# ctu-mrs/space_filling_forest_star

Measured on AMD Instinct MI355X. Metric: accepted node expansions/sec + collision checks/sec, dense_3D 6-DoF, higher is better.
Workload: dtype f64

## Files before the change

### space_filling_forest_star_amd/csrc/engine.cpp

```cpp
#include "engine.h"
#include <dlfcn.h>

#include <algorithm>
#include <chrono>
#include <cmath>
#include <cstdlib>
#include <cstring>
#include <limits>

#include "sff_geom.h"

namespace sff {

void hip_check(hipError_t e, const char* what) {
  if (e != hipSuccess) throw HipError{std::string(what) + ": " + hipGetErrorString(e)};
}
#define HIPCHK(x) hip_check((x), #x)

void DevBuf::ensure(size_t bytes) {
  if (bytes <= cap) return;
  size_t want = std::max(bytes, cap * 2);
  want = (want + 255) & ~(size_t)255;
  void* np = nullptr;
  HIPCHK(hipMalloc(&np, want));
// ... 142 lines not shown
  HIPCHK(hipEventCreateWithFlags(&ev_mid, hipEventDisableTiming));
  HIPCHK(hipEventCreateWithFlags(&ev_early, hipEventDisableTiming));
}

namespace {
struct RcclApi {
  struct Id128 { char b[128]; };
  int (*GetUniqueId)(void*) = nullptr;
  int (*CommInitRank)(void**, int, Id128, int) = nullptr;
  int (*AllGather)(const void*, void*, size_t, int, void*, hipStream_t) = nullptr;
  int (*CommDestroy)(void*) = nullptr;
  const char* (*GetErrorString)(int) = nullptr;
  bool ok = false;
};
RcclApi& rccl() {
  static RcclApi api;
  static bool tried = false;
  if (tried) return api;
  tried = true;
  void* h = nullptr;
  for (const char* name : {"librccl.so.1", "librccl.so"}) {
    h = dlopen(name, RTLD_NOW | RTLD_NOLOAD);
    if (h) break;
  }
  for (const char* name : {"librccl.so.1", "librccl.so", "/opt/rocm/lib/librccl.so.1"}) {
    if (h) break;
    h = dlopen(name, RTLD_NOW | RTLD_GLOBAL);
  }
  if (!h) return api;
  api.GetUniqueId = reinterpret_cast<decltype(api.GetUniqueId)>(dlsym(h, "ncclGetUniqueId"));
  api.CommInitRank = reinterpret_cast<decltype(api.CommInitRank)>(dlsym(h, "ncclCommInitRank"));
  api.AllGather = reinterpret_cast<decltype(api.AllGather)>(dlsym(h, "ncclAllGather"));
  api.CommDestroy = reinterpret_cast<decltype(api.CommDestroy)>(dlsym(h, "ncclCommDestroy"));
  api.GetErrorString = reinterpret_cast<decltype(api.GetErrorString)>(dlsym(h, "ncclGetErrorString"));
  api.ok = api.GetUniqueId && api.CommInitRank && api.AllGather && api.CommDestroy;
  return api;
}
void rccl_check(int rc, const char* what) {
  if (rc == 0) return;
  const char* msg = rccl().GetErrorString ? rccl().GetErrorString(rc) : "?";
  throw HipError{std::string("rccl: ") + what + " failed: " + msg};
}
}

void Ctx::rccl_unique_id(uint8_t* id128) {
  if (!rccl().ok) throw HipError{"rccl: librccl could not be bound"};
  rccl_check(rccl().GetUniqueId(id128), "ncclGetUniqueId");
}
void Ctx::rccl_init(const uint8_t* id128, int rank, int world) {
  if (!rccl().ok) throw HipError{"rccl: librccl could not be bound"};
  if (world < 1 || rank < 0 || rank >= world) throw HipError{"rccl: bad rank / world"};
  HIPCHK(hipSetDevice(device));
  if (rccl_comm) { (void)rccl().CommDestroy(rccl_comm); rccl_comm = nullptr; }
  RcclApi::Id128 id;
  memcpy(id.b, id128, 128);
  rccl_check(rccl().CommInitRank(&rccl_comm, world, id, rank), "ncclCommInitRank");
  rccl_rank = rank;
  rccl_world = world;
}
void Ctx::rccl_all_gather_i32(const void* send, void* recv, size_t words) {
  if (xchg_fn) {
    if (xchg_fn(xchg_user, send, recv, words, stream) != 0) throw HipError{"exchange: the caller's all-gather failed"};
    return;
  }
  rccl_check(rccl().AllGather(send, recv, words,  2, rccl_comm, stream), "ncclAllGather");
}

Ctx::~Ctx() {
  (void)hipSetDevice(device);
  if (stream) (void)hipStreamSynchronize(stream);
  if (own_stream && own_stream != stream) (void)hipStreamSynchronize(own_stream);
  if (copy_stream) (void)hipStreamSynchronize(copy_stream);
  if (rccl_comm && rccl().CommDestroy) { (void)rccl().CommDestroy(rccl_comm); rccl_comm = nullptr; }
  for (hipEvent_t e : rr_ev) if (e) (void)hipEventDestroy(e);
  for (SegJob& J : seg_job) if (J.ev) (void)hipEventDestroy(J.ev);
  if (ev_mid) (void)hipEventDestroy(ev_mid);
  if (ev_early) (void)hipEventDestroy(ev_early);
  for (auto& t : pending) { (void)hipEventDestroy(t.a); (void)hipEventDestroy(t.b); }
  for (auto e : pool) (void)hipEventDestroy(e);
  DevBuf* bufs[] = {&env_tri, &env_box, &env_plane, &rob_tri, &sx, &sy, &sz, &syaw, &spitch, &sroll, &stree, &spos,
                    &d_a, &d_b, &d_c, &d_d, &d_e, &d_f, &d_g, &d_h, &r_in, &r_out, &r_out2, &r_q, &r_cnt, &r_hidx,
                    &r_hdist, &r_sega, &r_segb, &r_items, &r_items2, &r_center, &r_qrec, &env_clear, &env_clear_edge, &env_cand, &g_cnt, &g_items, &g_ovfcnt, &g_ovf, &t_cnt, &t_items, &t_ovfcnt, &t_ovf, &t_occ, &g_lite, &g_ovf_lite, &t_lite, &t_ovf_lite, &env_tg_start, &env_tg_list, &r_sub, &env_ext, &rr_q1, &rr_q2, &rr_a, &rr_out, &rr_sq, &rr_np, &rr_alt, &rr_q2b, &rr_sqb, &seg_job[0].ids, &seg_job[0].a, &seg_job[0].b, &seg_job[0].c, &seg_job[1].ids, &seg_job[1].a,
                    &seg_job[1].b, &seg_job[1].c, &seg_job[2].ids, &seg_job[2].a, &seg_job[2].b, &seg_job[2].c, &seg_job[3].ids, &seg_job[3].a,
                    &seg_job[3].b, &seg_job[3].c};
  for (DevBuf* b : bufs) b->release();
  for (auto& b : level_box) b.release();
  PinBuf* pins[] = {&h_a, &h_b, &h_c, &h_d, &h_e, &h_f, &h_g, &h_h, &p_in, &p_out, &rr_hq, &rr_hout, &seg_job[0].hids, &seg_job[0].hc, &seg_job[1].hids, &seg_job[1].hc, &seg_job[2].hids, &seg_job[2].hc,
                    &seg_job[3].hids, &seg_job[3].hc};
  for (PinBuf* b : pins) b->release();
  if (copy_stream) (void)hipStreamDestroy(copy_stream);
  if (own_stream) (void)hipStreamDestroy(own_stream);
}

void Ctx::set_stream(hipStream_t s) {
  HIPCHK(hipSetDevice(device));
  sync();
  stream = s ? s : own_stream;
}

hipEvent_t Ctx::get_event() {
  if (!pool.empty()) {
    hipEvent_t e = pool.back();
    pool.pop_back();
    return e;
  }
  hipEvent_t e;
  HIPCHK(hipEventCreate(&e));
  return e;
}
void Ctx::time_begin(int kind) {
  kernel_calls[kind] += 1;
  if (round_scope) round_calls[kind] += 1;
  timed_now = timing_on;
  if (!timed_now) return;
  Timed t{get_event(), get_event(), kind, round_scope};
  HIPCHK(hipEventRecord(t.a, stream));
  pending.push_back(t);
}
void Ctx::time_end() { if (timed_now) HIPCHK(hipEventRecord(pending.back().b, stream)); }
double Ctx::kernel_ms_total(int kind) const {
  double ms = kernel_ms[kind];
  if (round_timed[kind]) ms += round_ms[kind] * ((double)round_calls[kind] / (double)round_timed[kind]);
  return ms;
}
void Ctx::sync() {
  HIPCHK(hipStreamSynchronize(stream));
  for (auto& t : pending) {
    float ms = 0;
    HIPCHK(hipEventElapsedTime(&ms, t.a, t.b));
    if (t.round) { round_ms[t.kind] += ms; round_timed[t.kind] += 1; }
    else kernel_ms[t.kind] += ms;
    kernel_launches[t.kind] += 1;
    pool.push_back(t.a);
    pool.push_back(t.b);
  }
  pending.clear();
}

static inline uint64_t spread21(uint64_t v) {
  v &= 0x1FFFFF;
  v = (v | v << 32) & 0x1F00000000FFFFULL;
  v = (v | v << 16) & 0x1F0000FF0000FFULL;
  v = (v | v << 8) & 0x100F00F00F00F00FULL;
  v = (v | v << 4) & 0x10C30C30C30C30C3ULL;
  v = (v | v << 2) & 0x1249249249249249ULL;
  return v;
}

void Ctx::upload_mesh(int role, const double* tri9, int n) {
  kn = Knobs::from_env();
  HIPCHK(hipSetDevice(device));
  if (role == SFFGPU_MESH_ROBOT) {
    if (n <= 0) throw HipError{"robot mesh must have at least one triangle"};
    rob_tri.ensure((size_t)n * 9 * sizeof(double));
    HIPCHK(hipMemcpy(rob_tri.p, tri9, (size_t)n * 9 * sizeof(double), hipMemcpyHostToDevice));
    robv.tri = rob_tri.as<double>();
    robv.n_tri = n;
    double lo[3] = {1e300, 1e300, 1e300}, hi[3] = {-1e300, -1e300, -1e300};
    for (int v = 0; v < n * 3; ++v)
      for (int i = 0; i < 3; ++i) {
        lo[i] = std::min(lo[i], tri9[3 * v + i]);
        hi[i] = std::max(hi[i], tri9[3 * v + i]);
      }
    double rad = 0;
    for (int i = 0; i < 3; ++i) { robv.lo[i] = lo[i]; robv.hi[i] = hi[i]; robv.center[i] = 0.5 * (lo[i] + hi[i]); }
    for (int v = 0; v < n * 3; ++v) {
      double d2 = 0;
      for (int i = 0; i < 3; ++i) d2 += (tri9[3 * v + i] - robv.center[i]) * (tri9[3 * v + i] - robv.center[i]);
      rad = std::max(rad, std::sqrt(d2));
    }
    robv.radius = rad;
    have_robot = true;
    h_rob.assign(tri9, tri9 + (size_t)n * 9);
    build_robot_extents();
    build_clearance();
    build_tri_grid();
    return;
  }
  if (role != SFFGPU_MESH_ENV) throw HipError{"unknown mesh role"};
  envv = sffk::EnvView{};
  have_env = true;
  clear_cells = 0;
  if (n <= 0) return;
  std::vector<double> box((size_t)n * 6);
  double glo[3] = {1e300, 1e300, 1e300}, ghi[3] = {-1e300, -1e300, -1e300};
  for (int t = 0; t < n; ++t)
    for (int a = 0; a < 3; ++a) {
      const double* P = tri9 + 9 * (size_t)t;
      double lo = std::min(P[a], std::min(P[3 + a], P[6 + a])), hi = std::max(P[a], std::max(P[3 + a], P[6 + a]));
      box[6 * (size_t)t + a] = lo;
      box[6 * (size_t)t + 3 + a] = hi;
      glo[a] = std::min(glo[a], lo);
      ghi[a] = std::max(ghi[a], hi);
    }
  for (int a = 0; a < 3; ++a) { env_lo[a] = glo[a]; env_hi[a] = ghi[a]; }
  env_maxabs = 1.0;
  for (int a = 0; a < 3; ++a) env_maxabs = std::max(env_maxabs, std::max(std::fabs(glo[a]), std::fabs(ghi[a])));
  std::vector<std::pair<uint64_t, int>> order(n);
  for (int t = 0; t < n; ++t) {
    uint64_t code = 0;
    for (int a = 0; a < 3; ++a) {
      double ext = ghi[a] - glo[a];
      double c = 0.5 * (box[6 * (size_t)t + a] + box[6 * (size_t)t + 3 + a]);
      double u = ext > 0 ? (c - glo[a]) / ext : 0.0;
      uint64_t q = (uint64_t)std::min(2097151.0, std::max(0.0, u * 2097151.0));
      code |= spread21(q) << a;
    }
    order[t] = {code, t};
  }
  std::sort(order.begin(), order.end());
  std::vector<double> tri_s((size_t)n * 9), box_s((size_t)n * 6);
  for (int k = 0; k < n; ++k) {
    memcpy(&tri_s[9 * (size_t)k], tri9 + 9 * (size_t)order[k].second, 9 * sizeof(double));
    memcpy(&box_s[6 * (size_t)k], &box[6 * (size_t)order[k].second], 6 * sizeof(double));
  }
  env_tri.ensure(tri_s.size() * sizeof(double));
  env_box.ensure(box_s.size() * sizeof(double));
  HIPCHK(hipMemcpy(env_tri.p, tri_s.data(), tri_s.size() * sizeof(double), hipMemcpyHostToDevice));
  HIPCHK(hipMemcpy(env_box.p, box_s.data(), box_s.size() * sizeof(double), hipMemcpyHostToDevice));
  std::vector<double> plane((size_t)n * 5);
  for (int k = 0; k < n; ++k) {
    const double* P = &tri_s[9 * (size_t)k];
    double e1[3] = {P[3] - P[0], P[4] - P[1], P[5] - P[2]}, e2[3] = {P[6] - P[0], P[7] - P[1], P[8] - P[2]}, nn[3];
    sffg::cross(e1, e2, nn);
    plane[5 * (size_t)k + 0] = nn[0];
    plane[5 * (size_t)k + 1] = nn[1];
    plane[5 * (size_t)k + 2] = nn[2];
    plane[5 * (size_t)k + 3] = (nn[0] * P[0] + nn[1] * P[1]) + nn[2] * P[2];
    plane[5 * (size_t)k + 4] = std::sqrt(nn[0] * nn[0] + nn[1] * nn[1] + nn[2] * nn[2]);
  }
  env_plane.ensure(plane.size() * sizeof(double));
  HIPCHK(hipMemcpy(env_plane.p, plane.data(), plane.size() * sizeof(double), hipMemcpyHostToDevice));
  envv.tri = env_tri.as<double>();
  envv.tri_box = env_box.as<double>();
  envv.tri_plane = env_plane.as<double>();
  envv.n_tri = n;
  h_plane = plane;
  std::vector<double> cur = box_s;
  int count = n, L = 0;
  while (true) {
    int groups = (count + 63) / 64;
    std::vector<double> nxt((size_t)groups * 6);
    for (int g = 0; g < groups; ++g) {
      double lo[3] = {1e300, 1e300, 1e300}, hi[3] = {-1e300, -1e300, -1e300};
      for (int k = g * 64; k < std::min(count, g * 64 + 64); ++k)
        for (int a = 0; a < 3; ++a) {
          lo[a] = std::min(lo[a], cur[6 * (size_t)k + a]);
          hi[a] = std::max(hi[a], cur[6 * (size_t)k + 3 + a]);
        }
      for (int a = 0; a < 3; ++a) { nxt[6 * (size_t)g + a] = lo[a]; nxt[6 * (size_t)g + 3 + a] = hi[a]; }
    }
    if (L >= SFFK_MAX_LEVELS) throw HipError{"environment mesh too large for the box hierarchy"};
    level_box[L].ensure(nxt.size() * sizeof(double));
    HIPCHK(hipMemcpy(level_box[L].p, nxt.data(), nxt.size() * sizeof(double), hipMemcpyHostToDevice));
    envv.level_box[L] = level_box[L].as<double>();
    envv.level_count[L] = groups;
    ++L;
    cur.swap(nxt);
    count = groups;
    if (groups <= 64) break;
  }
  envv.n_levels = L;
  build_robot_extents();
  build_clearance();
  build_tri_grid();
}

void Ctx::build_robot_extents() {
  envv.tri_ext = nullptr;
  envv.cand = nullptr;
  if (!have_env || !have_robot || envv.n_tri <= 0 || h_rob.empty() || h_plane.size() != (size_t)envv.n_tri * 5) return;
  std::vector<double> ext((size_t)envv.n_tri * 2);
  const size_t nv = h_rob.size() / 3;
  for (int k = 0; k < envv.n_tri; ++k) {
    const double* pl = &h_plane[5 * (size_t)k];
    double lo = 1e300, hi = -1e300;
    for (size_t v = 0; v < nv; ++v) {
      const double d = (pl[0] * h_rob[3 * v] + pl[1] * h_rob[3 * v + 1]) + pl[2] * h_rob[3 * v + 2];
      lo = std::min(lo, d);
      hi = std::max(hi, d);
    }
    ext[2 * (size_t)k] = lo;
    ext[2 * (size_t)k + 1] = hi;
  }
  env_ext.ensure(ext.size() * sizeof(double));
  HIPCHK(hipMemcpy(env_ext.p, ext.data(), ext.size() * sizeof(double), hipMemcpyHostToDevice));
  envv.tri_ext = env_ext.as<double>();
  std::vector<double> tb((size_t)envv.n_tri * 6), tt((size_t)envv.n_tri * 9), rec((size_t)envv.n_tri * 22);
  HIPCHK(hipMemcpy(tb.data(), env_box.p, tb.size() * sizeof(double), hipMemcpyDeviceToHost));
  HIPCHK(hipMemcpy(tt.data(), env_tri.p, tt.size() * sizeof(double), hipMemcpyDeviceToHost));
  for (int k = 0; k < envv.n_tri; ++k) {
    double* r = &rec[22 * (size_t)k];
    memcpy(r, &tb[6 * (size_t)k], 6 * sizeof(double));
    memcpy(r + 6, &h_plane[5 * (size_t)k], 5 * sizeof(double));
    memcpy(r + 11, &tt[9 * (size_t)k], 9 * sizeof(double));
    r[20] = ext[2 * (size_t)k];
    r[21] = ext[2 * (size_t)k + 1];
  }
  env_cand.ensure(rec.size() * sizeof(double));
  HIPCHK(hipMemcpy(env_cand.p, rec.data(), rec.size() * sizeof(double), hipMemcpyHostToDevice));
  envv.cand = env_cand.as<double>();
  if (kn.no_cand) envv.cand = nullptr;
}

void Ctx::build_clearance() {
  envv.clear_bits = nullptr;
  envv.clear_bits_edge = nullptr;
  clear_cells = 0;
  if (!have_env || !have_robot || envv.n_tri <= 0) return;
// ... 897 lines not shown
```

### space_filling_forest_star_amd/csrc/kernels.h

```cpp
#pragma once
#include <hip/hip_runtime.h>
#include <stdint.h>

#include "knobs.h"

namespace sffk {

struct NodeStoreView {
  const float* x;
  const float* y;
  const float* z;
  const float* yaw;
  const float* pitch;
  const float* roll;
  const int32_t* tree;
  const double* pos;
};

struct NodeStoreMut {
  float *x, *y, *z, *yaw, *pitch, *roll;
  int32_t* tree;
  double* pos;
};

struct SweepQuery {
  float x, y, z, yaw, pitch, roll;
  float r2f;
  int32_t tree;
  double r;
  int32_t max_id;
  int32_t active;
  int32_t pad, pad2;
};

struct GridItem {
  double p[6];
  int32_t id;
  int32_t tree;
  int32_t pad[2];
};
struct GridItem32 {
  float x, y, z, yaw, pitch, roll;
  int32_t id;
  int32_t tree;
};
struct GridView {
  float ox, oy, oz, inv_cell;
  int nx, ny, nz, bk;
  int32_t* cnt;
  GridItem* items;
  int32_t* ovf_cnt;
  GridItem* ovf;
  int ovf_cap;
  GridItem32* lite;
  GridItem32* ovf_lite;
  uint32_t* occ;
};

struct QRec {
  float q[6];
  float r2f;
  int32_t max_id;
  int32_t mine;
  int32_t evaluate;
  int32_t q_tree;
  int32_t total;
  int32_t lx, ly, lz;
  int32_t wx;
  int32_t ns0;
  float t0[6];
  int32_t wy;
  double pdist;
  double qr;
  int32_t scratch[4];
};
struct SampleParams {
  double limits[6];
  double dist_tree;
  double sweep_abs_eps;
  int rank, world;
};

#define SFFK_MAX_LEVELS 4
struct EnvView {
  const double* tri;
  const double* tri_box;
  const double* tri_plane;
  const double* tri_ext;
  const double* cand;
  int n_tri;
  int n_levels;
  const double* level_box[SFFK_MAX_LEVELS];
  int level_count[SFFK_MAX_LEVELS];
  const uint32_t* clear_bits;
  const uint32_t* clear_bits_edge;
  double clear_org[3];
  double clear_inv;
  int clear_n[3];
  const int32_t* tg_start;
  const int32_t* tg_list;
  double tg_org[3];
  double tg_inv;
  int tg_n[3];
};
void launch_tgrid_build(hipStream_t s, const EnvView& env, int32_t* cnt_or_start, int32_t* list, bool fill);
struct ClearBuildArgs {
  double thr_pose, thr_edge;
  double pose_lo[3], pose_hi[3];
  double edge_lo[3], edge_hi[3];
};
void launch_clear_build(hipStream_t s, const EnvView& env, const ClearBuildArgs& P, uint32_t* bits_pose, uint32_t* bits_edge,
                        long long n_cells);

struct RobotView {
  const double* tri;
  int n_tri;
  double center[3];
  double radius;
  double lo[3], hi[3];
};

struct DevCtrl {
  int32_t n_act;
  int32_t halt;
  int32_t n_nodes, iter, round, in_wave;
  int32_t n_slots, frontier_n, closed_n, use_closed;
  int32_t terminated, solved, empty_frontier, fault;
  int32_t N0, iter0, n_borders, n_unsettled;
  int32_t fault_pending, redraws, grid_ovf, tgrid_ovf;
  int32_t front_sel;
  int32_t compact_from;
  int32_t act_sel, act_cnt;
  int32_t app_n, app_N0, app_fn0, app_act_sel;
  int32_t iter0_app, app_act_cnt;
  int32_t claims_done;
  int32_t clear_n;
  unsigned long long cursor;
  unsigned long long words_base;
  unsigned long long collide_calls, path_free_calls, nn_queries;
  unsigned long long poses_executed, segments_executed, samples_executed;
  unsigned long long waves, rounds, round_nodes, round_queries;
  unsigned long long epoch;
  unsigned long long work_items;
  unsigned long long prof[8];
  unsigned long long q_t0, q_t1, q_ticks, q_launches;
  unsigned long long wprof[8];
  int32_t prio_n0, prio_wave, prio_all_empty, prio_gen;
  unsigned long long star_rounds, star_passes, star_members, star_rewires;
  int32_t ord_valid;
  int32_t app_nb0;
  int32_t status_seq, status_pad;
  unsigned long long spec_steps, spec_evaluated, spec_committed;
  int32_t spec_stalled, spec_pad;
};
#define SFFK_STATUS_RING 4
#define SFFK_DEV_MAX_GROUPS 1024
#define SFFK_FAULT_LISTS 1
#define SFFK_FAULT_BORDER_TABLE 2
#define SFFK_FAULT_CAPACITY 4
#define SFFK_FAULT_INTERNAL 16
#define SFFK_FAULT_PRIO_REDRAW 8

#define SFFK_ORD_BUCKETS 4096
#define SFFK_ORD_CNT_STRIDE 32
struct OrderView {
  int32_t* hist;
  int32_t* start;
  int32_t* slot_key;
  int32_t* slot_rank;
  int32_t* slot_pos;
  int32_t* lst[2];
  int32_t* cnt[2];
  int32_t n_sub;
  const double* pos;
  float ox, oy, oz, inv_cell;
  int32_t nx, ny, nz, shift, cnx, cny;
  int32_t n_buckets;
};

struct DevRound {
  const DevCtrl* ctrl;
  const int32_t* act_slot;
  const int32_t* act_slot2;
  const int32_t* slot_node;
  const uint8_t* nflag;
  const uint64_t* ring;
  uint64_t ring_mask;
  const double* trig;
  int32_t words_per;
  int32_t* parent_out;
  uint8_t* force_out;
  unsigned long long* qclk;
  unsigned long long* qclk_sh;
  OrderView ord;
};

struct RoundTemps {
  GridView tg;
  NodeStoreMut st;
  int32_t* cnt;
  int32_t* ctrl;
  int32_t* sub;
  int n_perm;
  int base;
  const double* preset;
  double* center_out;
  QRec* qrec;
  double clear_org[3];
  double clear_inv;
};

size_t collide_lds_bytes(int n_robot_tri, int waves);

void launch_sample_steer(hipStream_t s, const uint64_t* words, const int32_t* parent, const double* node_pos,
                         const double* center_in, int n, double dist, int dim, const SampleParams& prm, double* out6,
                         uint8_t* in_lim, double* parent_dist, SweepQuery* queries, int32_t q_max_base,
                         const RoundTemps& tmp, const DevRound* dev = nullptr);
struct SampleLaunch;
void launch_sample_steer(hipStream_t s, const SampleLaunch& P);

void launch_store_write(hipStream_t s, const NodeStoreMut& st, const double* pos6, const int32_t* tree,
                        const int32_t* parent, const uint8_t* active, int n, int base, const GridView* grid);

void launch_sweep(hipStream_t s, const NodeStoreView& st, int first, int n_nodes, const SweepQuery* queries,
                  const double* qpos, int nq, int32_t* cnt, int32_t* hit_idx, double* hit_dist, int cap);
void launch_grid_insert(hipStream_t s, const GridView& g, const NodeStoreView& st, int first, int n);
void launch_grid_query(hipStream_t s, const GridView& g, const GridView* tg, const NodeStoreView& st,
                       const SweepQuery* queries, const double* qpos, int nq, int32_t* cnt, int32_t* hit_idx,
                       double* hit_dist, int cap, const int32_t* dev_n = nullptr);
void launch_set_tree(hipStream_t s, int32_t* tree_col, const int32_t* ids, int n, int32_t value);

struct KnnQuery {
  double pos[6];
  int32_t tree;
  int32_t max_id;
  int32_t k;
  int32_t mate_base;
  int32_t whole_tree;
  int32_t pad_;
};
#define SFFK_KNN_MATES 64
void launch_knn_linear(hipStream_t s, const NodeStoreView& st, int n_store, const KnnQuery* q, int nq, int kcap,
                       int32_t* idx, double* dist, int32_t* cnt, double abs_eps);
void launch_rrt_steer(hipStream_t s, const KnnQuery* q1, const int32_t* idx1, int k1, const double* store_pos, double dist,
                      double* a6, double* np6, KnnQuery* q2, int kmax, int n, SweepQuery* sq, double sq_r, float sq_r2f,
                      double* np_copy, int32_t* seg_ns, int32_t* conn_cnt, const int32_t* alt_slot = nullptr,
                      const int32_t* alt_mate = nullptr, int row0 = 0);
void launch_rrt_alt_list(hipStream_t s, const int32_t* mate, int n, int cap, int32_t* alt_slot, int32_t* alt_mate, int32_t* cnt);
void launch_rrt_mates(hipStream_t s, const KnnQuery* q1, const double* near_d, int k1, const double* np6, const uint8_t* hit,
                      const int32_t* fh, const int32_t* ov, int n, int32_t* mate);
void launch_knn_grid(hipStream_t s, const GridView& g, const GridView* tg, const NodeStoreView& st, const KnnQuery* q, int nq,
                     int kcap, int32_t* idx, double* dist, int32_t* cnt, int32_t* mate_idx, int32_t* mate_cnt, double cell,
                     double slack, int mate_cap = SFFK_KNN_MATES, int n_store = 0);

void launch_collide_poses(hipStream_t s, const EnvView& env, const RobotView& rob, const double* pos6, int n,
                          const int32_t* live_flags, uint8_t* hit, bool explicit_rt = false);

struct ClassifyArgs {
  int n, N0, cap, nbcap, rank, world;
  int goal_id;
  double dist_tree;
  const double* newpos;
  const uint8_t* in_lim;
  const double* pdist;
  const int32_t* parent;
  const double* center;
  const uint8_t* force;
  const int32_t* cnt;
// ... 306 lines not shown
```

### space_filling_forest_star_amd/csrc/kernels.hip

```cpp
#include <hip/hip_runtime.h>
#include <stdint.h>
#include <stdlib.h>
#include <string.h>
#include "kernels.h"
#include <algorithm>
#include "sff_geom.h"
#include "kernels_dev.h"
#include "star_pass_dev.h"
#include "prio_heap_dev.h"

namespace sffk {

using namespace sffg;


__global__ __launch_bounds__(256) void k_sample_steer(SampleLaunch P) {
  const int i = blockIdx.x * blockDim.x + threadIdx.x;
  sample_steer_one(i, i, -1, P);
}

__device__ __forceinline__ float wrapf(float d) {
  const float PI_F = 3.14159274f;
  if (d < -PI_F) return d + 2.0f * PI_F;
  if (d >= PI_F) return d - 2.0f * PI_F;
// ... 3029 lines not shown
  auto settle = [&](bool need, int left, const uint32_t* wp, int sh, uint32_t word, int s, int t, int c) {
    const int gi = lane & 7;
    if (wp && ((word >> sh) & 1u)) need = false;
    unsigned long long m = need ? (((left >= 8 ? 0xffULL : ((1ULL << left) - 1ULL))) << (8 * gi)) : 0ULL;
    m |= __shfl_xor(m, 1);
    m |= __shfl_xor(m, 2);
    m |= __shfl_xor(m, 4);
    const bool lead = gi == 0 && m != 0ULL;
    if (lead) s_need[s][t] = 1;
    add_surv(lead, (int32_t)(s_map[s] * stride + t), c, m);
  };
  settle(e_s < S && e_need && s_i[e_s < S ? e_s : 0][QI_LIVE], e_left, e_wp, e_sh, e_word, e_s < S ? e_s : 0, 0, e_c);
  {
    const int tk_s = tid / QB_TASKS, tk_t = tid - tk_s * QB_TASKS;
    int nch = 0;
    if (tk_s < S && s_i[tk_s][QI_LIVE] && tk_t <= s_i[tk_s][QI_NNB]) {
      const int ns = s_NS[tk_s][tk_t];
      nch = ns > 0 ? (ns + 63) >> 6 : 0;
      if (tk_t == 0) nch = nch > 4 ? nch - 4 : 0;
    }
    int inc = nch;
    for (int off = 1; off < 64; off <<= 1) {
      const int o = __shfl_up(inc, off);
      if (lane >= off) inc += o;
    }
    if (lane == 63) s_wsum[wv] = inc;
    __syncthreads();
    int before = 0, P = 0;
    for (int w = 0; w < 4; ++w) { if (w < wv) before += s_wsum[w]; P += s_wsum[w]; }
    const int first = before + inc - nch;
    for (int w0 = 0; w0 < P; w0 += PAIRCAP) {
      if (w0) __syncthreads();
      for (int c = 0; c < nch; ++c) {
        const int p = first + c - w0;
        if (p >= 0 && p < PAIRCAP) s_tab[p] = (tk_s << 24) | (tk_t << 16) | ((tk_t == 0 ? 4 : 0) + c);
      }
      __syncthreads();
      const int wn = P - w0 < PAIRCAP ? P - w0 : PAIRCAP;
      for (int e0 = 0; e0 < 8 * wn; e0 += 256) {
        const int e = e0 + tid;
        const bool valid = e < 8 * wn;
        const int ent = valid ? s_tab[e >> 3] : 0;
        const int s = ent >> 24, t = (ent >> 16) & 0xff, c = ent & 0xffff;
        bool need;
        int left, sh;
        const uint32_t* wp;
        group_addr(valid, s_T[s][t], s_NS[s][t], c, tid & 7, need, left, wp, sh);
        const uint32_t word = wp ? *wp : 0u;
        settle(need, left, wp, sh, word, s, t, c);
      }
    }
  }
  if (tid < S) {
    const bool open = s_i[tid][QI_LIVE] && need_pose && !((word_pose >> sh_pose) & 1u);
    if (open) {
      const int at = atomicAdd(&s_cnt[2], 1);
      const SurvivorItem it{-1 - s_map[tid], 0, 0ULL};
      if (at < SURVCAP) s_surv[at] = it;
      else {
        SurvivorItem* list = static_cast<SurvivorItem*>(A.items);
        const int sub_list = blockIdx.x & (SFFK_SUBLISTS - 1), sub_cap = A.items_cap / SFFK_SUBLISTS, half = sub_cap / 2;
        const int p = atomicAdd(A.sub + sub_list * SFFK_SUB_STRIDE, 1);
        if (p < half) list[(size_t)sub_list * sub_cap + p] = it;
        else A.ctrl[3] = 1;
      }
    }
  }
  __syncthreads();
  QB_MARK(6);
  {
    const int ns = s_cnt[2] < SURVCAP ? s_cnt[2] : SURVCAP;
    if (wv == 0 && ns > 0) {
      SurvivorItem* list = static_cast<SurvivorItem*>(A.items);
      const int sub_list = blockIdx.x & (SFFK_SUBLISTS - 1), sub_cap = A.items_cap / SFFK_SUBLISTS, half = sub_cap / 2;
      for (int b0 = 0; b0 < ns; b0 += 64) {
        const bool mineb = b0 + lane < ns;
        const SurvivorItem it = mineb ? s_surv[b0 + lane] : SurvivorItem{0, 0, 0ULL};
        const bool hv = mineb && (it.slot < 0 || __popcll(it.mask) >= QC_HEAVY);
        const unsigned long long hm = __ballot(hv), lm = __ballot(mineb && !hv), below = (1ULL << lane) - 1ULL;
        int bh = 0, bl = 0;
        if (lane == 0) {
          if (hm) bh = atomicAdd(A.sub + sub_list * SFFK_SUB_STRIDE, __popcll(hm));
          if (lm) bl = atomicAdd(A.sub + sub_list * SFFK_SUB_STRIDE + 2, __popcll(lm));
        }
        bh = __shfl(bh, 0); bl = __shfl(bl, 0);
        if (hv) {
          const int at = bh + __popcll(hm & below);
          if (at < half) list[(size_t)sub_list * sub_cap + at] = it;
          else A.ctrl[3] = 1;
        } else if (mineb) {
          const int at = bl + __popcll(lm & below);
          if (at < sub_cap - half) list[(size_t)sub_list * sub_cap + half + at] = it;
          else A.ctrl[3] = 1;
        }
      }
    }
    const int tk_s = tid / QB_TASKS, tk_t = tid - tk_s * QB_TASKS;
    if (tk_s < S && s_need[tk_s][tk_t]) {
      const int i = s_map[tk_s];
      const size_t slot = (size_t)i * stride + tk_t;
      double* sa = A.seg_a + 6 * slot;
      double* sb = A.seg_b + 6 * slot;
      if (tk_t == 0) { for (int k = 0; k < 6; ++k) { sa[k] = s_ex[tk_s][k]; sb[k] = s_qp[tk_s][k]; } }
      else {
        const int hj = s_rankhit[tk_s][tk_t];
        const int id = h_id[tk_s][hj];
        const bool same = h_tree[tk_s][hj] == s_i[tk_s][QI_MINE];
        const double* nbp = A.pos + 6 * (size_t)id;
        if (same) { for (int k = 0; k < 6; ++k) { sa[k] = nbp[k]; sb[k] = s_qp[tk_s][k]; } }
        else if (id == A.goal_id) { for (int k = 0; k < 6; ++k) { sa[k] = s_qp[tk_s][k]; sb[k] = nbp[k]; } }
        else { for (int k = 0; k < 6; ++k) { sa[k] = s_ex[tk_s][k]; sb[k] = nbp[k]; } }
      }
    }
  }
  QB_MARK(7);
#ifdef SFFK_DEBUG_COUNTERS
  QDBG(10, clock64() - qb_c0); QDBG(11, wall_clock64() - qb_r0);
#endif
  if (clocked) {
    atomicMax(A.qclk_sh + (blockIdx.x & 63) * 16, wall_clock64());
  }
}

#ifndef CI_OCC
#define CI_OCC 2
#endif
template <bool SHARE>
__global__ __launch_bounds__(64 * SEG_WAVES) __attribute__((amdgpu_waves_per_eu(CI_OCC))) void k_collide_items(EnvView env, RobotView rob, const double* __restrict__ pos6,
                                                                  int n_pose, const int32_t* __restrict__ live_flags,
                                                                  uint8_t* __restrict__ pose_hit,
                                                                  const double* __restrict__ a6, const double* __restrict__ b6,
                                                                  const int32_t* __restrict__ seg_ns, int stride,
                                                                  int32_t* __restrict__ ctrl,
                                                                  const SurvivorItem* __restrict__ list, int items_cap,
                                                                  const int32_t* __restrict__ sub,
                                                                  int32_t* __restrict__ first_hit,
                                                                  int32_t* __restrict__ overflow_flag, GridView tg,
                                                                  const float* __restrict__ tx, const float* __restrict__ ty,
                                                                  const float* __restrict__ tz, int n_temps,
                                                                  const int32_t* __restrict__ dev_n, TaskSource D) {
#ifdef SFFK_CI_TRACE
  const unsigned long long ci_entry = wall_clock64();
#endif
  if (dev_n) {
    if (dev_n[1]) return;
    n_pose = dev_n[0];
    if (n_temps) n_temps = dev_n[0];
  }
  extern __shared__ double lds_d[];
  double* rtri = lds_d;
  const int wave = threadIdx.x >> 6, lane = threadIdx.x & 63;
  int sub_n = sub[lane * SFFK_SUB_STRIDE], sub_nl = sub[lane * SFFK_SUB_STRIDE + 2];
  const int ctrl3 = ctrl[3];
  constexpr int CI_PRE = 6;
  const int n9 = rob.n_tri * 9;
  double rv[CI_PRE];
#pragma unroll
  for (int k = 0; k < CI_PRE; ++k) {
    const int idx = (int)threadIdx.x + k * 256;
    rv[k] = idx < n9 ? rob.tri[idx] : 0.0;
  }
  const int gt0 = blockIdx.x * blockDim.x + threadIdx.x;
  float cx0 = __int_as_float(0x7fc00000), cy0 = 0.0f, cz0 = 0.0f;
  if (tg.cnt && gt0 < n_temps) { cx0 = tx[gt0]; cy0 = ty[gt0]; cz0 = tz[gt0]; }
#pragma unroll
  for (int k = 0; k < CI_PRE; ++k) {
    const int idx = (int)threadIdx.x + k * 256;
    if (idx < n9) rtri[idx] = rv[k];
  }
  for (int i = (int)threadIdx.x + CI_PRE * 256; i < n9; i += blockDim.x) rtri[i] = rob.tri[i];
  if (tg.cnt) {
    if (cx0 == cx0) {
      const size_t cell = grid_cell_of(tg, cx0, cy0, cz0);
      tg.cnt[cell] = 0;
      if (tg.occ) tg.occ[cell >> 5] = 0u;
    }
    for (int t = gt0 + gridDim.x * blockDim.x; t < n_temps; t += gridDim.x * blockDim.x) {
      const float x = tx[t];
      if (x == x) {
        const size_t cell = grid_cell_of(tg, x, ty[t], tz[t]);
        tg.cnt[cell] = 0;
        if (tg.occ) tg.occ[cell >> 5] = 0u;
      }
    }
    if (blockIdx.x == 0 && threadIdx.x == 0) tg.ovf_cnt[0] = 0;
  }
  double* stage = rtri + (size_t)rob.n_tri * 9 + (size_t)wave * STAGE_DOUBLES;
  int32_t* ibase = reinterpret_cast<int32_t*>(rtri + (size_t)rob.n_tri * 9 + (size_t)SEG_WAVES * STAGE_DOUBLES);
  const int sub_cap = items_cap / SFFK_SUBLISTS, sub_half = sub_cap / 2;
  sub_n = sub_n < sub_half ? sub_n : sub_half;
  sub_nl = sub_nl < sub_cap - sub_half ? sub_nl : sub_cap - sub_half;
  int sub_incl = sub_n, sub_incl_l = sub_nl;
  for (int off = 1; off < 64; off <<= 1) {
    const int o = __shfl_up(sub_incl, off), ol = __shfl_up(sub_incl_l, off);
    if (lane >= off) { sub_incl += o; sub_incl_l += ol; }
  }
  const int MH = __shfl(sub_incl, 63);
  const int M = MH + __shfl(sub_incl_l, 63);
  const bool ran_over = ctrl3 != 0;
  if (blockIdx.x == 0 && threadIdx.x == 0) ctrl[2] = M;
  if ((M <= 0 && !ran_over) || env.n_tri == 0) return;
  __shared__ ShareArea s_share;
  share_init(s_share);
  __syncthreads();
  double* rbox = reinterpret_cast<double*>(ibase + SEG_WAVES * (STACK_CAP + TG_HASH + CAND_CAP + QUEUE_CAP));
  fill_robot_boxes(rtri, rbox, rob.n_tri, threadIdx.x, blockDim.x);
  __syncthreads();
  int32_t* stack = ibase + wave * (STACK_CAP + TG_HASH);
  int32_t* cand = ibase + SEG_WAVES * (STACK_CAP + TG_HASH) + wave * CAND_CAP;
  int32_t* queue = ibase + SEG_WAVES * (STACK_CAP + TG_HASH + CAND_CAP) + wave * QUEUE_CAP;
  DBG_DECL
  const int W = gridDim.x * SEG_WAVES;
#ifdef SFFK_CI_TRACE
  const unsigned long long ci_t0 = ci_entry, ci_pre = wall_clock64();
  const unsigned int ci_seen = __hip_atomic_load(&g_ci_launch, __ATOMIC_RELAXED, __HIP_MEMORY_SCOPE_AGENT);
  const bool ci_on = ci_seen == SFFK_CI_TRACE;
  int ci_items = 0;
  unsigned long long ci_first[4] = {0, 0, 0, 0};
#endif
  const int n_slots = n_pose * stride;
  const int E = ran_over ? n_pose + n_slots : M;
  int32_t* const ticket = const_cast<int32_t*>(sub) + (size_t)((blockIdx.x + gridDim.x * wave) & (SFFK_SUBLISTS - 1)) * SFFK_SUB_STRIDE + 1;
  auto next_item = [&](int e) -> int {
    if (ran_over) return e + W;
    int t = 0;
    if (lane == 0) t = atomicAdd(ticket, 1);
    t = __builtin_amdgcn_readfirstlane(t);
    return W + ((blockIdx.x + gridDim.x * wave) & (SFFK_SUBLISTS - 1)) + SFFK_SUBLISTS * t;
  };
  for (int e = blockIdx.x + gridDim.x * wave; e < E; e = next_item(e)) {
    int slot, c_lo, c_hi;
    unsigned long long mask = 0ULL;
    if (!ran_over) {
      size_t at;
      if (e < MH) {
        const int sl = __popcll(__ballot(sub_incl <= e));
        at = (size_t)sl * sub_cap + (e - (__shfl(sub_incl, sl) - __shfl(sub_n, sl)));
      } else {
        const int e2 = e - MH;
        const int sl = __popcll(__ballot(sub_incl_l <= e2));
        at = (size_t)sl * sub_cap + sub_half + (e2 - (__shfl(sub_incl_l, sl) - __shfl(sub_nl, sl)));
      }
      const SurvivorItem it = list[at];
      slot = it.slot; c_lo = it.chunk; c_hi = it.chunk + 1; mask = it.mask;
    } else if (e < n_pose) {
      if ((live_flags[e] & 3) != 1) continue;
      slot = -1 - e; c_lo = c_hi = 0;
    } else {
      slot = e - n_pose;
      if (D.on) {
        const int si = slot / stride;
        if ((live_flags[si] & 3) != 1 || slot - si * stride > D.rec_nnb[si]) continue;
      }
      const int ns = seg_ns[slot];
      if (ns <= 0) continue;
      c_lo = 0; c_hi = (ns + 63) >> 6;
    }
    if (slot < 0) {
      const int pose = -1 - slot;
      double p[6], R[9], c[3];
#ifdef SFFK_CI_TRACE
      const unsigned long long ci_p0 = wall_clock64();
#endif
      pose_frame(rob, pos6, pose, p, R, c);
      const bool hit = pose_exact(env, rob, rtri, stack, cand, stage, p, R, c, lane, (SHARE && !ran_over) ? &s_share : nullptr);
      if (lane == 0) pose_hit[pose] = hit ? 1 : 0;
#ifdef SFFK_CI_TRACE
      ci_first[3] += ((wall_clock64() - ci_p0) << 8) | 1ULL;
#endif
      continue;
    }
    double a[6], b[6];
    if (D.on && ran_over) {
      const int si = slot / stride, t = slot - si * stride;
      const double* pe = D.center ? D.center + 6 * (size_t)si : D.pos + 6 * (size_t)D.parent[si];
      const double* pq = pos6 + 6 * (size_t)si;
      if (t == 0) { for (int k = 0; k < 6; ++k) { a[k] = pe[k]; b[k] = pq[k]; } }
      else {
        const int id = D.rec_nb[(size_t)si * D.nbcap + t - 1];
        const bool same = (D.rec_meta[(size_t)si * D.nbcap + t - 1] & 1) != 0;
        const double* pn = D.pos + 6 * (size_t)id;
        if (same) { for (int k = 0; k < 6; ++k) { a[k] = pn[k]; b[k] = pq[k]; } }
        else if (id == D.goal_id) { for (int k = 0; k < 6; ++k) { a[k] = pq[k]; b[k] = pn[k]; } }
        else { for (int k = 0; k < 6; ++k) { a[k] = pe[k]; b[k] = pn[k]; } }
      }
    } else {
      for (int k = 0; k < 6; ++k) { a[k] = a6[6 * (size_t)slot + k]; b[k] = b6[6 * (size_t)slot + k]; }
    }
    for (int chunk = c_lo; chunk < c_hi; ++chunk) {
      if (chunk > 0 && first_hit[slot] <= 64 * chunk) break;
#ifdef SFFK_CI_TRACE
      const unsigned long long ci_a = wall_clock64();
#endif
      segment_chunk(env, rob, rtri, rbox, stack, cand, queue, stage, a, b, slot, chunk, !ran_over, mask, first_hit, overflow_flag, lane DBG_PASS,
                            (SHARE && !ran_over) ? &s_share : nullptr);
#ifdef SFFK_CI_TRACE
      if (ci_items == 0) { ci_first[0] = ci_a; ci_first[1] = wall_clock64(); ci_first[2] = (unsigned long long)__popcll(mask); }
      ++ci_items;
#endif
    }
  }
  if (SHARE) share_help(env, rob, rtri, rbox, queue, stage, ibase + SEG_WAVES * (STACK_CAP + TG_HASH), s_share, lane DBG_PASS);
#ifdef SFFK_CI_TRACE
  if (ci_on && lane == 0) {
    const int gw = (blockIdx.x * blockDim.x + threadIdx.x) >> 6;
    unsigned long long* o = g_ci_trace + 8 * (size_t)gw;
    o[0] = ci_t0; o[1] = ci_first[0]; o[2] = ci_items ? g_ci_tmp[2 * gw] : 0ULL; o[3] = ci_first[1];
    o[4] = ci_items ? g_ci_tmp[2 * gw + 1] : 0ULL; o[5] = ci_first[2] | (ci_pre << 8); o[6] = (unsigned long long)ci_items | (ci_first[3] << 8); o[7] = wall_clock64();
  }
  if (blockIdx.x == 0 && threadIdx.x == 0) atomicAdd(&g_ci_launch, 1u);
#endif
  DBG_FLUSH();
}

struct ExactLds {
  double* rtri; double* rbox; double* stage; int32_t* stack; int32_t* cand; int32_t* queue; int32_t* cand_base;
};
__device__ __forceinline__ ExactLds exact_lds(double* lds_d, int n_rob_tri, int wave) {
  ExactLds E;
  E.rtri = lds_d;
  E.stage = E.rtri + (size_t)n_rob_tri * 9 + (size_t)wave * STAGE_DOUBLES;
  int32_t* ibase = reinterpret_cast<int32_t*>(E.rtri + (size_t)n_rob_tri * 9 + (size_t)SEG_WAVES * STAGE_DOUBLES);
  E.rbox = reinterpret_cast<double*>(ibase + SEG_WAVES * (STACK_CAP + TG_HASH + CAND_CAP + QUEUE_CAP));
  E.stack = ibase + wave * (STACK_CAP + TG_HASH);
  E.cand_base = ibase + SEG_WAVES * (STACK_CAP + TG_HASH);
  E.cand = E.cand_base + wave * CAND_CAP;
  E.queue = ibase + SEG_WAVES * (STACK_CAP + TG_HASH + CAND_CAP) + wave * QUEUE_CAP;
  return E;
}
template <bool COH>
__device__ __forceinline__ void star_exact_items(const EnvView& env, const RobotView& rob, const ExactLds& E,
                                                 const double* __restrict__ store_pos, const int32_t* ida,
                                                 const int32_t* idb, const SurvivorItem* list,
                                                 int sub_cap, int32_t* sub, int sub_n, int sub_incl, int M,
                                                 int32_t* first_hit, int32_t* overflow_flag,
                                                 ShareArea& s_share, int wg, int nwg, int wave, int lane) {
  DBG_DECL
  const int W = nwg * SEG_WAVES;
  const bool few = W < SFFK_SUBLISTS;
  const int grp = few ? 0 : ((wg + nwg * wave) & (SFFK_SUBLISTS - 1));
  int32_t* const ticket = sub + (size_t)grp * SFFK_STAR_SUB + 1;
  auto next_item = [&]() -> int {
    int t = 0;
    if (lane == 0) t = atomicAdd(ticket, 1);
    t = __builtin_amdgcn_readfirstlane(t);
    return few ? W + t : W + grp + SFFK_SUBLISTS * t;
  };
  for (int e = wg + nwg * wave; e < M; e = next_item()) {
    const int sl = __popcll(__ballot(sub_incl <= e));
    const int j = e - (__shfl(sub_incl, sl) - __shfl(sub_n, sl));
    const SurvivorItem it = sld<COH>(list + (size_t)sl * sub_cap + j);
    const int slot = it.slot;
    if (it.chunk > 0 && sld<COH>(first_hit + slot) <= 64 * it.chunk) continue;
    double a[6], b[6];
    const double* pa = store_pos + 6 * (size_t)sld<COH>(ida + slot);
    const double* pb = store_pos + 6 * (size_t)sld<COH>(idb + slot);
    for (int k = 0; k < 6; ++k) { a[k] = pa[k]; b[k] = pb[k]; }
    segment_chunk(env, rob, E.rtri, E.rbox, E.stack, E.cand, E.queue, E.stage, a, b, slot, it.chunk, true, it.mask, first_hit,
                  overflow_flag, lane DBG_PASS, &s_share);
  }
  share_help(env, rob, E.rtri, E.rbox, E.queue, E.stage, E.cand_base, s_share, lane DBG_PASS);
}

__global__ __launch_bounds__(64 * SEG_WAVES) __attribute__((amdgpu_waves_per_eu(CI_OCC))) void k_star_exact(
    EnvView env, RobotView rob, const double* __restrict__ store_pos, const int32_t* __restrict__ ida,
    const int32_t* __restrict__ idb, const SurvivorItem* __restrict__ list, int items_cap, int32_t* __restrict__ sub,
    int32_t* __restrict__ first_hit, int32_t* __restrict__ overflow_flag, int32_t* __restrict__ hdr) {
  const int wave = threadIdx.x >> 6, lane = threadIdx.x & 63;
  int sub_n = sub[lane * SFFK_STAR_SUB];
  const int h_skip = hdr[1], h_fault = hdr[4];
  if (h_skip || h_fault) return;
  extern __shared__ double lds_d[];
  const ExactLds E = exact_lds(lds_d, rob.n_tri, wave);
  const int sub_cap = items_cap / SFFK_SUBLISTS;
  if (sub_n > sub_cap) {
    if (blockIdx.x == 0 && wave == 0) atomicOr(hdr + 4, 1);
    sub_n = sub_cap;
  }
  int sub_incl = sub_n;
  for (int off = 1; off < 64; off <<= 1) {
    const int o = __shfl_up(sub_incl, off);
    if (lane >= off) sub_incl += o;
  }
  const int M = __shfl(sub_incl, 63);
  if (M <= 0 || env.n_tri == 0) return;
  __shared__ ShareArea s_share;
  share_init(s_share);
  for (int i = threadIdx.x; i < rob.n_tri * 9; i += blockDim.x) E.rtri[i] = rob.tri[i];
  __syncthreads();
  fill_robot_boxes(E.rtri, E.rbox, rob.n_tri, threadIdx.x, blockDim.x);
  __syncthreads();
  star_exact_items<false>(env, rob, E, store_pos, ida, idb, list, sub_cap, sub, sub_n, sub_incl, M, first_hit, overflow_flag, s_share,
                          blockIdx.x, gridDim.x, wave, lane);
}

#define STAR_BAR_TICKS 4000000ULL
__device__ __forceinline__ void star_decide(int32_t* s_dec, const int32_t* fault, const int32_t* chg) {
  __syncthreads();
  if (threadIdx.x == 0) {
    s_dec[0] = __hip_atomic_load(fault, __ATOMIC_RELAXED, __HIP_MEMORY_SCOPE_AGENT);
    s_dec[1] = chg ? __hip_atomic_load(chg, __ATOMIC_RELAXED, __HIP_MEMORY_SCOPE_AGENT) : 0;
  }
  __syncthreads();
}
__device__ __forceinline__ void star_grid_barrier(int32_t* bar, int target, int32_t* fault, unsigned long long* dbg) {
  __builtin_amdgcn_fence(__ATOMIC_RELEASE, "workgroup");
  __builtin_amdgcn_s_waitcnt(0);
  __syncthreads();
  if (threadIdx.x == 0) {
    const unsigned long long ta = wall_clock64();
    __hip_atomic_fetch_add(bar, 1, __ATOMIC_RELAXED, __HIP_MEMORY_SCOPE_AGENT);
    const unsigned long long t0 = wall_clock64();
    while (__hip_atomic_load(bar, __ATOMIC_RELAXED, __HIP_MEMORY_SCOPE_AGENT) < target) {
      __builtin_amdgcn_s_sleep(2);
      if (wall_clock64() - t0 > STAR_BAR_TICKS) { atomicOr(fault, 1); break; }
    }
    const unsigned long long t1 = wall_clock64();
    if (dbg) { const unsigned long long t2 = wall_clock64(); dbg[0] += t0 - ta; dbg[1] += t1 - t0; dbg[2] += t2 - t1; }
  }
  __syncthreads();
}

__global__ __launch_bounds__(64 * SEG_WAVES) __attribute__((amdgpu_waves_per_eu(CI_OCC))) void k_star_tail(
    ResolveArgs A, EnvView env, RobotView rob, NodeStoreView st, int max_passes, int test_stall) {
  __shared__ StarPassLds L;
  __shared__ ShareArea s_share;
  __shared__ int32_t s_dec[2];
  extern __shared__ double lds_d[];
  const DevForestView& f = A.f;
  const StarView& S = A.S;
  const DevCtrl* c = f.ctrl;
  const int app_n = c->app_n, N0 = c->app_N0;
  const unsigned ep = (unsigned)c->epoch;
  const int h_n = S.hdr[0], h_skip = S.hdr[1], n_ev = S.hdr[2], ev_first = S.hdr[3], h_fault = S.hdr[STAR_FAULT];
  const int chg0 = S.changed[0];
  if (app_n <= 0 || h_skip || h_fault) return;
  const int wg = blockIdx.x, wave = threadIdx.x >> 6, lane = threadIdx.x & 63;
  if (chg0 == 0 || max_passes <= 1) {
    if (wg == 0 && threadIdx.x == 0) { S.hdr[STAR_PASSES_RUN] = 1; S.hdr[STAR_CONVERGED] = chg0 == 0; }
    return;
  }
  int g_act = (h_n + 3) >> 2;
  g_act = g_act < 16 ? 16 : g_act;
  g_act = g_act > (int)gridDim.x ? (int)gridDim.x : g_act;
  if (wg >= g_act) return;
  if (test_stall > 0 && g_act > 1 && wg == g_act - 1 && ep % (unsigned)test_stall == 0u) return;
  const int Tb = f.temp_base;
  const ExactLds E = exact_lds(lds_d, rob.n_tri, wave);
  const int sub_cap = S.items_cap / SFFK_SUBLISTS;
  int32_t* const bar = S.changed + SFFK_STAR_BAR;
  int32_t* const fault = S.hdr + STAR_FAULT;
  bool robot_ready = false, conv = false;
  int n_bar = 0, pass = 1;
  unsigned long long* const dbg = (S.dbg && wg == 0) ? S.dbg + 16 : nullptr;
  unsigned long long tp = dbg ? wall_clock64() : 0ULL;
// ... 2006 lines not shown
```

Before: 11.23 million.

## Precompute robot triangle boxes on host and defer temp-grid cleanup to kernel end

Robot triangle AABBs are now computed once on the host and uploaded right after the triangle data. The collision kernel stages them straight into LDS instead of running fill_robot_boxes with an extra barrier on every launch. The temp-grid counter clearing and the ctrl[2] write move to a lambda that runs at kernel exit, which takes global stores off the startup critical path. A shuffle is also swapped for readlane. The risk is ordering: other blocks may read the grid cells or the control word before the deferred clear has happened.

Result: no change. 11.15 million (-0.7%).

```diff
diff --git a/space_filling_forest_star_amd/csrc/engine.cpp b/space_filling_forest_star_amd/csrc/engine.cpp
--- a/space_filling_forest_star_amd/csrc/engine.cpp
+++ b/space_filling_forest_star_amd/csrc/engine.cpp
@@ -318,9 +318,17 @@
   HIPCHK(hipSetDevice(device));
   if (role == SFFGPU_MESH_ROBOT) {
     if (n <= 0) throw HipError{"robot mesh must have at least one triangle"};
-    rob_tri.ensure((size_t)n * 9 * sizeof(double));
-    HIPCHK(hipMemcpy(rob_tri.p, tri9, (size_t)n * 9 * sizeof(double), hipMemcpyHostToDevice));
+    std::vector<double> tri15((size_t)n * 15);
+    std::copy(tri9, tri9 + (size_t)n * 9, tri15.begin());
+    for (int r = 0; r < n; ++r)
+      for (int ax = 0; ax < 3; ++ax) {
+        tri15[(size_t)n * 9 + 6 * r + ax] = sffg::min3(tri9[9 * r + ax], tri9[9 * r + 3 + ax], tri9[9 * r + 6 + ax]);
+        tri15[(size_t)n * 9 + 6 * r + 3 + ax] = sffg::max3(tri9[9 * r + ax], tri9[9 * r + 3 + ax], tri9[9 * r + 6 + ax]);
+      }
+    rob_tri.ensure(tri15.size() * sizeof(double));
+    HIPCHK(hipMemcpy(rob_tri.p, tri15.data(), tri15.size() * sizeof(double), hipMemcpyHostToDevice));
     robv.tri = rob_tri.as<double>();
+    robv.tri_box = robv.tri + (size_t)n * 9;
     robv.n_tri = n;
     double lo[3] = {1e300, 1e300, 1e300}, hi[3] = {-1e300, -1e300, -1e300};
     for (int v = 0; v < n * 3; ++v)
diff --git a/space_filling_forest_star_amd/csrc/kernels.h b/space_filling_forest_star_amd/csrc/kernels.h
--- a/space_filling_forest_star_amd/csrc/kernels.h
+++ b/space_filling_forest_star_amd/csrc/kernels.h
@@ -114,6 +114,7 @@
 
 struct RobotView {
   const double* tri;
+  const double* tri_box;
   int n_tri;
   double center[3];
   double radius;
diff --git a/space_filling_forest_star_amd/csrc/kernels.hip b/space_filling_forest_star_amd/csrc/kernels.hip
--- a/space_filling_forest_star_amd/csrc/kernels.hip
+++ b/space_filling_forest_star_amd/csrc/kernels.hip
@@ -3205,41 +3205,31 @@
   const int wave = threadIdx.x >> 6, lane = threadIdx.x & 63;
   int sub_n = sub[lane * SFFK_SUB_STRIDE], sub_nl = sub[lane * SFFK_SUB_STRIDE + 2];
   const int ctrl3 = ctrl[3];
-  constexpr int CI_PRE = 6;
-  const int n9 = rob.n_tri * 9;
+  constexpr int CI_PRE = 8;
+  const int n9 = rob.n_tri * 9, n15 = rob.n_tri * 15;
   double rv[CI_PRE];
 #pragma unroll
   for (int k = 0; k < CI_PRE; ++k) {
     const int idx = (int)threadIdx.x + k * 256;
-    rv[k] = idx < n9 ? rob.tri[idx] : 0.0;
+    rv[k] = idx < n15 ? rob.tri[idx] : 0.0;
   }
   const int gt0 = blockIdx.x * blockDim.x + threadIdx.x;
   float cx0 = __int_as_float(0x7fc00000), cy0 = 0.0f, cz0 = 0.0f;
   if (tg.cnt && gt0 < n_temps) { cx0 = tx[gt0]; cy0 = ty[gt0]; cz0 = tz[gt0]; }
+  double* stage = rtri + (size_t)rob.n_tri * 9 + (size_t)wave * STAGE_DOUBLES;
+  int32_t* ibase = reinterpret_cast<int32_t*>(rtri + (size_t)rob.n_tri * 9 + (size_t)SEG_WAVES * STAGE_DOUBLES);
+  double* rbox = reinterpret_cast<double*>(ibase + SEG_WAVES * (STACK_CAP + TG_HASH + CAND_CAP + QUEUE_CAP));
 #pragma unroll
   for (int k = 0; k < CI_PRE; ++k) {
     const int idx = (int)threadIdx.x + k * 256;
     if (idx < n9) rtri[idx] = rv[k];
-  }
-  for (int i = (int)threadIdx.x + CI_PRE * 256; i < n9; i += blockDim.x) rtri[i] = rob.tri[i];
-  if (tg.cnt) {
-    if (cx0 == cx0) {
-      const size_t cell = grid_cell_of(tg, cx0, cy0, cz0);
-      tg.cnt[cell] = 0;
-      if (tg.occ) tg.occ[cell >> 5] = 0u;
-    }
-    for (int t = gt0 + gridDim.x * blockDim.x; t < n_temps; t += gridDim.x * blockDim.x) {
-      const float x = tx[t];
-      if (x == x) {
-        const size_t cell = grid_cell_of(tg, x, ty[t], tz[t]);
-        tg.cnt[cell] = 0;
-        if (tg.occ) tg.occ[cell >> 5] = 0u;
-      }
-    }
-    if (blockIdx.x == 0 && threadIdx.x == 0) tg.ovf_cnt[0] = 0;
-  }
-  double* stage = rtri + (size_t)rob.n_tri * 9 + (size_t)wave * STAGE_DOUBLES;
-  int32_t* ibase = reinterpret_cast<int32_t*>(rtri + (size_t)rob.n_tri * 9 + (size_t)SEG_WAVES * STAGE_DOUBLES);
+    else if (idx < n15) rbox[idx - n9] = rv[k];
+  }
+  for (int i = (int)threadIdx.x + CI_PRE * 256; i < n15; i += blockDim.x) {
+    const double v = rob.tri[i];
+    if (i < n9) rtri[i] = v; else rbox[i - n9] = v;
+  }
+  const int cell0 = cx0 == cx0 ? (int)grid_cell_of(tg, cx0, cy0, cz0) : -1;
   const int sub_cap = items_cap / SFFK_SUBLISTS, sub_half = sub_cap / 2;
   sub_n = sub_n < sub_half ? sub_n : sub_half;
   sub_nl = sub_nl < sub_cap - sub_half ? sub_nl : sub_cap - sub_half;
@@ -3248,16 +3238,30 @@
     const int o = __shfl_up(sub_incl, off), ol = __shfl_up(sub_incl_l, off);
     if (lane >= off) { sub_incl += o; sub_incl_l += ol; }
   }
-  const int MH = __shfl(sub_incl, 63);
-  const int M = MH + __shfl(sub_incl_l, 63);
+  const int MH = __builtin_amdgcn_readlane(sub_incl, 63);
+  const int M = MH + __builtin_amdgcn_readlane(sub_incl_l, 63);
   const bool ran_over = ctrl3 != 0;
-  if (blockIdx.x == 0 && threadIdx.x == 0) ctrl[2] = M;
-  if ((M <= 0 && !ran_over) || env.n_tri == 0) return;
+  auto clean_up = [&]() {
+    if (tg.cnt) {
+      if (cell0 >= 0) {
+        tg.cnt[cell0] = 0;
+        if (tg.occ) tg.occ[cell0 >> 5] = 0u;
+      }
+      for (int t = gt0 + gridDim.x * blockDim.x; t < n_temps; t += gridDim.x * blockDim.x) {
+        const float x = tx[t];
+        if (x == x) {
+          const size_t cell = grid_cell_of(tg, x, ty[t], tz[t]);
+          tg.cnt[cell] = 0;
+          if (tg.occ) tg.occ[cell >> 5] = 0u;
+        }
+      }
+      if (blockIdx.x == 0 && threadIdx.x == 0) tg.ovf_cnt[0] = 0;
+    }
+    if (blockIdx.x == 0 && threadIdx.x == 0) ctrl[2] = M;
+  };
+  if ((M <= 0 && !ran_over) || env.n_tri == 0) { clean_up(); return; }
   __shared__ ShareArea s_share;
   share_init(s_share);
-  __syncthreads();
-  double* rbox = reinterpret_cast<double*>(ibase + SEG_WAVES * (STACK_CAP + TG_HASH + CAND_CAP + QUEUE_CAP));
-  fill_robot_boxes(rtri, rbox, rob.n_tri, threadIdx.x, blockDim.x);
   __syncthreads();
   int32_t* stack = ibase + wave * (STACK_CAP + TG_HASH);
   int32_t* cand = ibase + SEG_WAVES * (STACK_CAP + TG_HASH) + wave * CAND_CAP;
@@ -3354,6 +3358,7 @@
     }
   }
   if (SHARE) share_help(env, rob, rtri, rbox, queue, stage, ibase + SEG_WAVES * (STACK_CAP + TG_HASH), s_share, lane DBG_PASS);
+  clean_up();
 #ifdef SFFK_CI_TRACE
   if (ci_on && lane == 0) {
     const int gw = (blockIdx.x * blockDim.x + threadIdx.x) >> 6;
```
